# elfi-dev/elfi

Hardware: NVIDIA H100
Metric: accepted particles/sec (higher is better)
Workload: dtype f64

## Files before the change

### elfi_b200/csrc/common.cuh

```cuda
#pragma once

#include <cuda.h>
#include <cuda_runtime.h>

#include <cstdarg>
#include <cstdint>
#include <cstdio>
#include <cstring>

#include "../../include/elfi_b200.h"

namespace elfi {

void set_error(const char* fmt, ...);

#define ELFI_CUDA_OK(expr)                                                              \
    do {                                                                                \
        cudaError_t _e = (expr);                                                        \
        if (_e != cudaSuccess) {                                                        \
            ::elfi::set_error("%s failed: %s (%s:%d)", #expr, cudaGetErrorString(_e),   \
                              __FILE__, __LINE__);                                      \
            cudaGetLastError();       \
            return ELFI_B200_ERR_CUDA;                                                  \
        }                                                                               \
// ... 8 lines not shown
    } while (0)

typedef CUresult (*tensor_map_encode_fn)(CUtensorMap*, CUtensorMapDataType, cuuint32_t, void*,
                                         const cuuint64_t*, const cuuint64_t*,
                                         const cuuint32_t*, const cuuint32_t*,
                                         CUtensorMapInterleave, CUtensorMapSwizzle,
                                         CUtensorMapL2promotion, CUtensorMapFloatOOBfill);

}

struct elfi_b200_ctx {
    int device;
    int sm_count;
    size_t smem_optin;
    elfi::tensor_map_encode_fn encode_tiled;
    void* scratch;
    size_t scratch_bytes;
    void* pinned;
    size_t pinned_bytes;
    void* dev_stage;
    size_t dev_stage_bytes;
    cudaStream_t copy_stream[2];
    cudaEvent_t copy_event[4];
};

namespace elfi {

void* ctx_scratch(elfi_b200_ctx* ctx, size_t bytes);

int make_rowmajor_f64_map(elfi_b200_ctx* ctx, const double* base, int64_t rows, int64_t cols,
                          int64_t ld, int box_rows, CUtensorMap* out);

inline bool tma_compatible(const void* base, int64_t ld) {
    return (reinterpret_cast<uintptr_t>(base) % 16 == 0) && ((ld * 8) % 16 == 0);
}

__device__ __forceinline__ uint32_t smem_u32(const void* p) {
    return static_cast<uint32_t>(__cvta_generic_to_shared(p));
}

__device__ __forceinline__ void mbar_init(uint32_t bar, uint32_t count) {
    asm volatile("mbarrier.init.shared::cta.b64 [%0], %1;" ::"r"(bar), "r"(count) : "memory");
}

__device__ __forceinline__ void mbar_fence_init() {
    asm volatile("fence.mbarrier_init.release.cluster;" ::: "memory");
// ... 25 lines not shown
}

__device__ __forceinline__ void tma_load_2d(uint32_t dst, const CUtensorMap* map, int32_t col0,
                                            int32_t row0, uint32_t bar) {
    asm volatile(
        "cp.async.bulk.tensor.2d.shared::cluster.global.mbarrier::complete_tx::bytes"
        " [%0], [%1, {%2, %3}], [%4];"
        ::"r"(dst), "l"(reinterpret_cast<uint64_t>(map)), "r"(col0), "r"(row0), "r"(bar)
        : "memory");
}

__device__ __forceinline__ void bulk_load_1d(uint32_t dst, const void* src, uint32_t bytes,
                                             uint32_t bar) {
    asm volatile(
        "cp.async.bulk.shared::cluster.global.mbarrier::complete_tx::bytes [%0], [%1], %2, [%3];"
        ::"r"(dst), "l"(src), "r"(bytes), "r"(bar)
        : "memory");
}

__device__ __forceinline__ void tma_prefetch_desc(const CUtensorMap* map) {
    asm volatile("prefetch.tensormap [%0];" ::"l"(reinterpret_cast<uint64_t>(map)) : "memory");
}

}
```

### elfi_b200/csrc/ctx.cu

```cuda
#include "common.cuh"

namespace elfi {

static thread_local char g_error[512] = "";

void set_error(const char* fmt, ...) {
    va_list ap;
    va_start(ap, fmt);
    vsnprintf(g_error, sizeof(g_error), fmt, ap);
    va_end(ap);
}

void* ctx_scratch(elfi_b200_ctx* ctx, size_t bytes) {
    if (bytes <= ctx->scratch_bytes) return ctx->scratch;
    size_t want = bytes + (bytes >> 2) + (1u << 20);
    want = (want + 255) & ~size_t(255);
    if (ctx->scratch) {
        if (cudaDeviceSynchronize() != cudaSuccess || cudaFree(ctx->scratch) != cudaSuccess) {
            set_error("scratch release failed: %s", cudaGetErrorString(cudaGetLastError()));
            ctx->scratch = nullptr;
            ctx->scratch_bytes = 0;
            return nullptr;
        }
        ctx->scratch = nullptr;
// ... 54 lines not shown
        elfi::set_error("ctx_create: device %d is sm_%d%d; this library is built for sm_90a only",
                        device, prop.major, prop.minor);
        return ELFI_B200_ERR_UNSUPPORTED;
    }
    elfi_b200_ctx* ctx = new elfi_b200_ctx();
    memset(ctx, 0, sizeof(*ctx));
    ctx->device = device;
    ctx->sm_count = prop.multiProcessorCount;
    ctx->smem_optin = prop.sharedMemPerBlockOptin;
    void* fn = nullptr;
    cudaDriverEntryPointQueryResult qres;
    cudaError_t e = cudaGetDriverEntryPoint("cuTensorMapEncodeTiled", &fn, cudaEnableDefault, &qres);
    if (e != cudaSuccess || qres != cudaDriverEntryPointSuccess || fn == nullptr) {
        elfi::set_error("ctx_create: cuTensorMapEncodeTiled not available from the driver");
        delete ctx;
        cudaGetLastError();
        return ELFI_B200_ERR_CUDA;
    }
    ctx->encode_tiled = reinterpret_cast<elfi::tensor_map_encode_fn>(fn);
    for (int i = 0; i < 2; ++i)
        ELFI_CUDA_OK(cudaStreamCreateWithFlags(&ctx->copy_stream[i], cudaStreamNonBlocking));
    for (int i = 0; i < 4; ++i)
        ELFI_CUDA_OK(cudaEventCreateWithFlags(&ctx->copy_event[i], cudaEventDisableTiming));
    *out = ctx;
    return ELFI_B200_OK;
}

int elfi_b200_ctx_destroy(elfi_b200_ctx* ctx) {
    if (!ctx) return ELFI_B200_OK;
    cudaSetDevice(ctx->device);
    cudaDeviceSynchronize();
    if (ctx->scratch) cudaFree(ctx->scratch);
    if (ctx->dev_stage) cudaFree(ctx->dev_stage);
    if (ctx->pinned) cudaFreeHost(ctx->pinned);
    for (int i = 0; i < 2; ++i)
        if (ctx->copy_stream[i]) cudaStreamDestroy(ctx->copy_stream[i]);
    for (int i = 0; i < 4; ++i)
        if (ctx->copy_event[i]) cudaEventDestroy(ctx->copy_event[i]);
    delete ctx;
    return ELFI_B200_OK;
}

int elfi_b200_ctx_sm_count(const elfi_b200_ctx* ctx) { return ctx ? ctx->sm_count : 0; }

int elfi_b200_allgather_particles(elfi_b200_ctx* const* ctxs, int64_t n_ctx, const double* const* send,
                                  int64_t rows, int64_t width, double* const* recv,
                                  void* const* streams) {
    ELFI_REQUIRE(ctxs && send && recv && streams && n_ctx >= 1 && n_ctx <= 64,
                 "allgather_particles: bad argument");
    ELFI_REQUIRE(rows >= 0 && width >= 1, "allgather_particles: bad shape");
    for (int64_t g = 0; g < n_ctx; ++g)
        ELFI_REQUIRE(ctxs[g] && (rows == 0 || (send[g] && recv[g])), "allgather_particles: NULL entry %lld",
                     (long long)g);
    if (rows == 0) return ELFI_B200_OK;
    const size_t bytes = size_t(rows) * size_t(width) * 8;
    int caller_device = 0;
    ELFI_CUDA_OK(cudaGetDevice(&caller_device));
// ... 43 lines not shown
```

### elfi_b200/csrc/distance.cu

```cuda
#include <cstdlib>

#include "rowstream.cuh"

extern "C" int elfi_b200_colmoments_f64(elfi_b200_ctx* ctx, const double* S, int64_t ldS, int64_t B,
                                        int64_t D, double* out, void* stream);

namespace elfi {

struct DistParams {
    const double* obs;
    const double* W;
    double* d_out;
    uint32_t* mask;
    int K;
    int has_thr;
    const double* shift_src;
    double* mom_partial;
    const double* thr_dev;
    double thr[ELFI_B200_MAX_NESTED];
    __device__ __forceinline__ double threshold(int k) const {
        return thr_dev ? __ldg(thr_dev + k) : thr[k];
    }
};

// ... 294 lines not shown
                for (int j = 0; j < D; ++j) {
                    const double d = __dsub_rn(__ldg(r + j), __ldg(p.obs + j));
                    acc = __dadd_rn(acc, __dmul_rn(__ldg(w + j), __dmul_rn(d, d)));
                }
            } else {
                for (int j = 0; j < D; ++j) {
                    const double d = __dsub_rn(__ldg(r + j), __ldg(p.obs + j));
                    acc = __dadd_rn(acc, __dmul_rn(d, d));
                }
            }
            const double dist = sqrt(acc);
            p.d_out[row * K + k] = dist;
            if (p.has_thr) ok = ok && (dist <= p.threshold(k));
        }
    }
    if (p.mask != nullptr) {
        const uint32_t bits = __ballot_sync(0xffffffffu, ok && p.has_thr);
        if (lane == 0 && (row - lane) < B) p.mask[row >> 5] = bits;
    }
}

__global__ void __launch_bounds__(1024)
compact_mask_kernel(const uint32_t* __restrict__ mask, int64_t nwords, int64_t B,
                    int32_t* __restrict__ idx, int64_t* __restrict__ n_out) {
    __shared__ int64_t warp_sums[32];
    __shared__ int64_t base_s;
    const int tid = threadIdx.x;
    const int lane = tid & 31;
    const int wid = tid >> 5;
    const int64_t first = int64_t(blockIdx.x) * 1024;

    int64_t before = 0;
    for (int64_t w = tid; w < first; w += 1024) before += __popc(mask[w]);
    for (int o = 16; o > 0; o >>= 1) before += __shfl_xor_sync(0xffffffffu, before, o);
    if (lane == 0) warp_sums[wid] = before;
    __syncthreads();
    if (tid == 0) {
        int64_t t = 0;
        for (int i = 0; i < 32; ++i) t += warp_sums[i];
        base_s = t;
    }
    __syncthreads();
    const int64_t base = base_s;
    __syncthreads();

    const int64_t w = first + tid;
    const uint32_t bits = w < nwords ? mask[w] : 0u;
    const int cnt = __popc(bits);
    int incl = cnt;
    for (int o = 1; o < 32; o <<= 1) {
        const int t = __shfl_up_sync(0xffffffffu, incl, o);
        if (lane >= o) incl += t;
    }
    if (lane == 31) warp_sums[wid] = incl;
    __syncthreads();
    if (wid == 0) {
        int64_t v = warp_sums[lane];
        int64_t inc2 = v;
        for (int o = 1; o < 32; o <<= 1) {
            const int64_t t = __shfl_up_sync(0xffffffffu, inc2, o);
            if (lane >= o) inc2 += t;
        }
        warp_sums[lane] = inc2 - v;
        if (lane == 31 && blockIdx.x == gridDim.x - 1 && n_out != nullptr) *n_out = base + inc2;
    }
    __syncthreads();
    int64_t pos = base + warp_sums[wid] + (incl - cnt);
    if (idx != nullptr) {
        uint32_t b = bits;
        while (b) {
            const int bit = __ffs(b) - 1;
            b &= b - 1;
            idx[pos++] = int32_t(w * 32 + bit);
        }
    }
}

int launch_compact_mask(const uint32_t* mask, int64_t B, int32_t* idx, int64_t* n_out,
                        cudaStream_t stream) {
    const int64_t nwords = (B + 31) / 32;
    if (nwords == 0) {
        if (n_out) ELFI_CUDA_OK(cudaMemsetAsync(n_out, 0, sizeof(int64_t), stream));
        return ELFI_B200_OK;
    }
    const unsigned blocks = unsigned((nwords + 1023) / 1024);
    compact_mask_kernel<<<blocks, 1024, 0, stream>>>(mask, nwords, B, idx, n_out);
    ELFI_CUDA_OK(cudaGetLastError());
    return ELFI_B200_OK;
}

int launch_dist(elfi_b200_ctx* ctx, const double* S, int64_t ldS, int64_t B, int64_t D,
                const double* obs, const double* W, int64_t K, const double* thr_host,
                double* d_out, uint32_t* mask, cudaStream_t stream,
                const double* thr_dev = nullptr) {
    DistParams p;
    memset(&p, 0, sizeof(p));
    p.obs = obs;
    p.W = W;
    p.d_out = d_out;
    p.mask = mask;
    p.K = int(K);
    p.has_thr = thr_host != nullptr || thr_dev != nullptr;
    p.thr_dev = thr_dev;
    if (thr_host)
        for (int k = 0; k < K; ++k) p.thr[k] = thr_host[k];
    if (B == 0) return ELFI_B200_OK;

    const int64_t Dp = ((D + RS_BOX_COLS - 1) / RS_BOX_COLS) * RS_BOX_COLS;
    const bool use_tma = D >= RS_BOX_COLS && tma_compatible(S, ldS);
    if (use_tma) {
// ... 243 lines not shown
    const int64_t Dp = ((D + RS_BOX_COLS - 1) / RS_BOX_COLS) * RS_BOX_COLS;
    const size_t aux = size_t(Dp) * 8 * 2;
    if (D >= RS_BOX_COLS && tma_compatible(S, ldS) && rs_pick_stages(ctx->smem_optin, aux) >= 2)
        return rowstream_launch<SeuclidConsumer>(ctx, S, ldS, B, D, aux, p, stream);
    seuclid_direct_kernel<<<unsigned((B + 255) / 256), 256, 0, stream>>>(S, ldS, B, int(D), p);
    ELFI_CUDA_OK(cudaGetLastError());
    return ELFI_B200_OK;
}

static int check_dist_args(const void* S, int64_t ldS, int64_t B, int64_t D, const void* obs,
                           const void* W, int64_t K, const void* thr, const void* acc_idx) {
    ELFI_REQUIRE(B >= 0 && D >= 1, "dist: bad shape B=%lld D=%lld", (long long)B, (long long)D);
    ELFI_REQUIRE(B == 0 || S != nullptr, "dist: S is NULL");
    ELFI_REQUIRE(obs != nullptr, "dist: obs is NULL");
    ELFI_REQUIRE(ldS >= D, "dist: ldS (%lld) < D (%lld)", (long long)ldS, (long long)D);
    ELFI_REQUIRE(K >= 1 && K <= ELFI_B200_MAX_NESTED, "dist: K=%lld outside [1, %d]",
                 (long long)K, ELFI_B200_MAX_NESTED);
    ELFI_REQUIRE(W != nullptr || K == 1, "dist: K=%lld needs a weight matrix", (long long)K);
    ELFI_REQUIRE(acc_idx == nullptr || thr != nullptr, "dist: acc_idx requires thresholds");
    ELFI_REQUIRE(B < (int64_t(1) << 31), "dist: B must fit int32 row indices");
    return ELFI_B200_OK;
}

}

extern "C" {

int elfi_b200_dist_euclid_thr_f64(elfi_b200_ctx* ctx, const double* S, int64_t ldS, int64_t B,
                                  int64_t D, const double* obs, const double* W, int64_t K,
                                  const double* thr_host, double* d_out, int32_t* acc_idx,
                                  int64_t* n_acc, void* stream_) {
    using namespace elfi;
    ELFI_REQUIRE(ctx != nullptr, "dist: ctx is NULL");
    int rc = check_dist_args(S, ldS, B, D, obs, W, K, thr_host, acc_idx);
    if (rc) return rc;
    ELFI_REQUIRE(B == 0 || d_out != nullptr, "dist: d_out is NULL");
    cudaStream_t stream = static_cast<cudaStream_t>(stream_);
    ELFI_CUDA_OK(cudaSetDevice(ctx->device));
    uint32_t* mask = nullptr;
    if (thr_host != nullptr) {
        const size_t nwords = size_t((B + 31) / 32);
        mask = static_cast<uint32_t*>(ctx_scratch(ctx, nwords * 4 + 256));
        if (!mask) return ELFI_B200_ERR_NOMEM;
    }
    rc = launch_dist(ctx, S, ldS, B, D, obs, W, K, thr_host, d_out, mask, stream);
    if (rc) return rc;
    if (thr_host != nullptr && (acc_idx != nullptr || n_acc != nullptr))
        return launch_compact_mask(mask, B, acc_idx, n_acc, stream);
    return ELFI_B200_OK;
}

int elfi_b200_dist_euclid_thr_dev_f64(elfi_b200_ctx* ctx, const double* S, int64_t ldS, int64_t B,
                                      int64_t D, const double* obs, const double* W, int64_t K,
                                      const double* thr_dev, double* d_out, int32_t* acc_idx,
                                      int64_t* n_acc, void* stream_) {
    using namespace elfi;
    ELFI_REQUIRE(ctx != nullptr && thr_dev != nullptr, "dist: ctx or thr_dev is NULL");
    int rc = check_dist_args(S, ldS, B, D, obs, W, K, thr_dev, acc_idx);
    if (rc) return rc;
    ELFI_REQUIRE(B == 0 || d_out != nullptr, "dist: d_out is NULL");
    cudaStream_t stream = static_cast<cudaStream_t>(stream_);
    ELFI_CUDA_OK(cudaSetDevice(ctx->device));
    const size_t nwords = size_t((B + 31) / 32);
    uint32_t* mask = static_cast<uint32_t*>(ctx_scratch(ctx, nwords * 4 + 256));
    if (!mask) return ELFI_B200_ERR_NOMEM;
    rc = launch_dist(ctx, S, ldS, B, D, obs, W, K, nullptr, d_out, mask, stream, thr_dev);
    if (rc) return rc;
    if (acc_idx != nullptr || n_acc != nullptr)
        return launch_compact_mask(mask, B, acc_idx, n_acc, stream);
    return ELFI_B200_OK;
}

int elfi_b200_dist_euclid_mom_f64(elfi_b200_ctx* ctx, const double* S, int64_t ldS, int64_t B,
                                  int64_t D, const double* obs, const double* W, int64_t K,
                                  const double* thr_host, const double* thr_dev, double* d_out,
                                  int32_t* acc_idx, int64_t* n_acc, double* moments,
                                  void* stream_) {
    using namespace elfi;
    ELFI_REQUIRE(ctx != nullptr && moments != nullptr, "dist_mom: ctx or moments is NULL");
    ELFI_REQUIRE(!(thr_host && thr_dev), "dist_mom: give thresholds on the host OR on the device");
    const void* thr = thr_host ? static_cast<const void*>(thr_host) : thr_dev;
    int rc = check_dist_args(S, ldS, B, D, obs, W, K, thr, acc_idx);
    if (rc) return rc;
    ELFI_REQUIRE(B >= 1 && d_out != nullptr, "dist_mom: needs at least one row and d_out");
    cudaStream_t stream = static_cast<cudaStream_t>(stream_);
    ELFI_CUDA_OK(cudaSetDevice(ctx->device));
    const int64_t Dp = ((D + RS_BOX_COLS - 1) / RS_BOX_COLS) * RS_BOX_COLS;
    const size_t aux = NestedMomentsConsumer<2>::aux_bytes(Dp, K);
    const bool fused = W != nullptr && D >= RS_BOX_COLS && tma_compatible(S, ldS) &&
                       rs_pick_stages(ctx->smem_optin, aux) >= 2;
    const size_t mask_bytes = (size_t((B + 31) / 32) * 4 + 255) & ~size_t(255);
    const size_t part_bytes = fused ? size_t(ctx->sm_count) * 16 * 2 * D * 8 : 0;
    uint8_t* base = static_cast<uint8_t*>(ctx_scratch(ctx, mask_bytes + part_bytes + 256));
// ... 178 lines not shown
```

### elfi_b200/csrc/rowstream.cuh

```cuda
#pragma once

#include <type_traits>

#include "common.cuh"

namespace elfi {

template <class C, class = void> struct rs_has_tile_info : std::false_type {};
template <class C> struct rs_has_tile_info<C, std::void_t<decltype(C::RS_TILE_INFO)>> : std::true_type {};
template <class C, class = void> struct rs_has_finish : std::false_type {};
template <class C> struct rs_has_finish<C, std::void_t<decltype(C::RS_FINISH)>> : std::true_type {};

constexpr int RS_WARPS = 8;
constexpr int RS_BOX_ROWS = 32;
constexpr int RS_BOX_COLS = 16;
constexpr int RS_BOX_BYTES = RS_BOX_ROWS * RS_BOX_COLS * 8;
constexpr int RS_MAX_STAGES = 6;

__host__ __device__ inline size_t rs_box_bytes(int ns, int warps = RS_WARPS) {
    return size_t(warps) * ns * RS_BOX_BYTES;
}
__host__ __device__ inline size_t rs_bar_bytes(int ns, int warps = RS_WARPS) {
    return size_t(warps) * ns * 8;
}
__host__ __device__ inline size_t rs_aux_offset(int ns, int warps = RS_WARPS) {
    return (rs_box_bytes(ns, warps) + rs_bar_bytes(ns, warps) + 15) & ~size_t(15);
}

inline int rs_pick_stages(size_t smem_optin, size_t aux_bytes, int warps = RS_WARPS) {
    for (int ns = RS_MAX_STAGES; ns >= 2; --ns)
        if (rs_aux_offset(ns, warps) + aux_bytes + 1024 <= smem_optin) return ns;
    return 0;
}

template <class Consumer, int WARPS = RS_WARPS>
__global__ void __launch_bounds__(WARPS * 32, 1)
rowstream_kernel(const __grid_constant__ CUtensorMap map, int64_t B, int D, int ns,
                 typename Consumer::Params params) {
    extern __shared__ __align__(1024) uint8_t smem[];
    const int warp = threadIdx.x >> 5;
    const int lane = threadIdx.x & 31;
    uint8_t* aux = smem + rs_aux_offset(ns, WARPS);

    Consumer::setup_shared(aux, params, D);

    const uint32_t box0 = smem_u32(smem) + uint32_t(warp) * ns * RS_BOX_BYTES;
    const uint32_t bar0 = smem_u32(smem + rs_box_bytes(ns, WARPS)) + uint32_t(warp) * ns * 8;
    const uint8_t* box0_generic = smem + size_t(warp) * ns * RS_BOX_BYTES;

    if (lane == 0) {
        if (warp == 0) tma_prefetch_desc(&map);
        for (int s = 0; s < ns; ++s) mbar_init(bar0 + s * 8, 1);
        mbar_fence_init();
    }
    __syncthreads();

    const int Gc = (D + RS_BOX_COLS - 1) / RS_BOX_COLS;
    const int G = Gc * Consumer::PASSES;
    const int64_t ntiles = (B + RS_BOX_ROWS - 1) / RS_BOX_ROWS;
    const int64_t gw = int64_t(blockIdx.x) * WARPS + warp;
    const int64_t GW = int64_t(gridDim.x) * WARPS;
    const int64_t my_tiles = gw < ntiles ? (ntiles - gw + GW - 1) / GW : 0;
    const int64_t nbox = my_tiles * G;

    int64_t p_tile = gw;
    int p_cg = 0;
    int p_col = 0;
    int64_t p_q = 0;
    int p_s = 0;
    auto issue = [&]() {
        mbar_arrive_expect_tx(bar0 + p_s * 8, RS_BOX_BYTES);
        tma_load_2d(box0 + p_s * RS_BOX_BYTES, &map, p_col * RS_BOX_COLS,
                    int32_t(p_tile * RS_BOX_ROWS), bar0 + p_s * 8);
        ++p_q;
        if (++p_s == ns) p_s = 0;
        if (++p_col == Gc) p_col = 0;
        if (++p_cg == G) { p_cg = 0; p_tile += GW; }
// ... 7 lines not shown
    const int sw = lane & 7;
    const uint32_t row_off = uint32_t(lane) * 128;

    int s = 0;
    uint32_t parity = 0;
    int cg = 0;
    int col = 0;
    int pass = 0;
    int64_t tile = gw;
    for (int64_t q = 0; q < nbox; ++q) {
        mbar_wait(bar0 + s * 8, parity);
        if (cg == 0) {
            c.begin_row();
            if constexpr (rs_has_tile_info<Consumer>::value) c.set_tile(tile * RS_BOX_ROWS, B);
        }
        c.consume(pass, col, box0_generic + size_t(s) * RS_BOX_BYTES + row_off, sw);
        __syncwarp();
        if (lane == 0 && p_q < nbox) issue();
        if (cg == G - 1) c.end_row(tile * RS_BOX_ROWS + lane, B, lane);
        if (++col == Gc) { col = 0; ++pass; }
        if (++cg == G) { cg = 0; pass = 0; tile += GW; }
        if (++s == ns) { s = 0; parity ^= 1; }
    }
    if constexpr (rs_has_finish<Consumer>::value) {
        __syncwarp();
        c.finish(gw, lane);
    }
}

template <class Consumer, int WARPS = RS_WARPS>
int rowstream_launch(elfi_b200_ctx* ctx, const double* M, int64_t ld, int64_t B, int64_t D,
                     size_t aux_bytes, const typename Consumer::Params& params,
                     cudaStream_t stream) {
    ELFI_REQUIRE(D <= (int64_t(1) << 30) && B < (int64_t(1) << 31),
                 "matrix too large for int32 TMA coordinates (B=%lld, D=%lld)", (long long)B,
                 (long long)D);
    if (B == 0) return ELFI_B200_OK;
    const int ns = rs_pick_stages(ctx->smem_optin, aux_bytes, WARPS);
    ELFI_REQUIRE(ns >= 2, "row too wide for the shared-memory pipeline (D=%lld)", (long long)D);
    CUtensorMap map;
    int rc = make_rowmajor_f64_map(ctx, M, B, D, ld, RS_BOX_ROWS, &map);
    if (rc) return rc;
    const size_t smem_bytes = rs_aux_offset(ns, WARPS) + aux_bytes;
    auto kern = rowstream_kernel<Consumer, WARPS>;
    ELFI_CUDA_OK(cudaFuncSetAttribute(kern, cudaFuncAttributeMaxDynamicSharedMemorySize,
                                      int(smem_bytes)));
    const int64_t ntiles = (B + RS_BOX_ROWS - 1) / RS_BOX_ROWS;
    int64_t ctas = (ntiles + WARPS - 1) / WARPS;
    if (ctas > ctx->sm_count) ctas = ctx->sm_count;
    kern<<<dim3(unsigned(ctas)), dim3(WARPS * 32), smem_bytes, stream>>>(map, B, int(D), ns, params);
    ELFI_CUDA_OK(cudaGetLastError());
    return ELFI_B200_OK;
}

}
```

### elfi_b200/csrc/select.cu

```cuda
#include <cstdlib>

#include "eqweight.h"
#include "pairwise.cuh"

namespace elfi {

constexpr int SORT_CHUNK = 1024;
constexpr int SORT_WARPS = 8;

__device__ __forceinline__ uint64_t key_to_u64(double d) {
    if (d != d) return ~uint64_t(0);
    uint64_t u = static_cast<uint64_t>(__double_as_longlong(d));
    return (u >> 63) ? ~u : (u | (uint64_t(1) << 63));
}
__device__ __forceinline__ double u64_to_key(uint64_t u) {
    if (u == ~uint64_t(0)) return __longlong_as_double(0x7ff8000000000000LL);
    u = (u >> 63) ? (u & ~(uint64_t(1) << 63)) : ~u;
    return __longlong_as_double(static_cast<long long>(u));
}

__global__ void __launch_bounds__(256)
sort_prepare_kernel(const double* __restrict__ keys, int64_t n, uint64_t* __restrict__ ukeys,
                    int32_t* __restrict__ vals, uint32_t* __restrict__ ghist) {
    __shared__ uint32_t h[8 * 256];
// ... 164 lines not shown
    int cur = 0;
    for (int pass = 0; pass < 8; ++pass) {
        sort_upsweep_kernel<<<wblocks, SORT_WARPS * 32, 0, stream>>>(s.k[cur], n, pass, s.nw, s.ghist, s.whist);
        sort_scan_kernel<<<256, 1024, 0, stream>>>(s.k[cur], n, pass, s.nw, s.ghist, s.whist);
        sort_scatter_kernel<<<wblocks, SORT_WARPS * 32, 0, stream>>>(
            s.k[cur], s.v[cur], n, pass, s.nw, s.ghist, s.whist, s.k[cur ^ 1], s.v[cur ^ 1]);
        cur ^= 1;
    }
    ELFI_CUDA_OK(cudaGetLastError());
    return ELFI_B200_OK;
}

__global__ void __launch_bounds__(256)
gather_rows_kernel(const double* __restrict__ src, int64_t ld_src, const int32_t* __restrict__ idx,
                   int64_t n, int64_t width, double* __restrict__ dst, int64_t ld_dst) {
    const int64_t total = n * width;
    const int64_t stride = int64_t(gridDim.x) * blockDim.x;
    for (int64_t t = int64_t(blockIdx.x) * blockDim.x + threadIdx.x; t < total; t += stride) {
        const int64_t i = t / width, j = t - i * width;
        dst[i * ld_dst + j] = src[int64_t(idx[i]) * ld_src + j];
    }
}

constexpr int APPEND_MAX_SRC = 8;
struct AppendSources {
    const double* ptr[APPEND_MAX_SRC];
    int64_t ld[APPEND_MAX_SRC];
    int32_t width[APPEND_MAX_SRC];
    int32_t col0[APPEND_MAX_SRC];
    int32_t n_src, total_width;
};

__global__ void __launch_bounds__(256)
accept_append_kernel(const int32_t* __restrict__ acc_idx, const int64_t* __restrict__ n_acc,
                     AppendSources src, double* __restrict__ dst, int64_t ld_dst, int64_t capacity,
                     const int64_t* __restrict__ count) {
    const int64_t base = *count;
    int64_t room = capacity - base;
    if (room < 0) room = 0;
    const int64_t rows = *n_acc < room ? *n_acc : room;
    const int64_t total = rows * src.total_width;
    const int64_t stride = int64_t(gridDim.x) * blockDim.x;
    for (int64_t t = int64_t(blockIdx.x) * blockDim.x + threadIdx.x; t < total; t += stride) {
        const int64_t j = t / src.total_width;
        const int c = int(t - j * src.total_width);
        const int64_t row = acc_idx ? int64_t(acc_idx[j]) : j;
        int k = 0;
#pragma unroll
        for (int q = 1; q < APPEND_MAX_SRC; ++q)
            if (q < src.n_src && c >= src.col0[q]) k = q;
        dst[(base + j) * ld_dst + c] = src.ptr[k][row * src.ld[k] + (c - src.col0[k])];
    }
}

__global__ void accept_count_kernel(const int64_t* __restrict__ n_acc, int64_t capacity,
                                    int64_t* __restrict__ count, int64_t* __restrict__ dropped) {
    int64_t room = capacity - *count;
    if (room < 0) room = 0;
    const int64_t rows = *n_acc < room ? *n_acc : room;
    if (dropped) *dropped += *n_acc - rows;
    *count += rows;
}

__global__ void __launch_bounds__(256)
gather2_rows_kernel(const double* __restrict__ A, int64_t ldA, int64_t nA,
                    const double* __restrict__ Bm, int64_t ldB, const int32_t* __restrict__ mapB,
                    const int32_t* __restrict__ perm, int64_t n, int64_t width,
                    double* __restrict__ dst, int64_t ld_dst) {
    const int64_t total = n * width;
    const int64_t stride = int64_t(gridDim.x) * blockDim.x;
    for (int64_t t = int64_t(blockIdx.x) * blockDim.x + threadIdx.x; t < total; t += stride) {
        const int64_t i = t / width, j = t - i * width;
        const int64_t r = perm ? perm[i] : i;
        double v;
        if (r < nA) {
            v = A[r * ldA + j];
        } else {
            const int64_t rb = mapB ? int64_t(mapB[r - nA]) : (r - nA);
            v = Bm[rb * ldB + j];
        }
        dst[i * ld_dst + j] = v;
    }
}

// ... 482 lines not shown
        const int64_t width = width_host[k];
        ELFI_REQUIRE(width >= 1 && dst_host[k] && ld_dst_host[k] >= width &&
                     (nA == 0 || (A_host[k] && ldA_host[k] >= width)) &&
                     (nB == 0 || (B_host[k] && ldB_host[k] >= width)),
                     "topn_merge: bad descriptor of output %lld", (long long)k);
        int64_t gb = (n_keep * width + 255) / 256;
        if (gb > int64_t(ctx->sm_count) * 16) gb = int64_t(ctx->sm_count) * 16;
        gather2_rows_kernel<<<unsigned(gb), 256, 0, stream>>>(A_host[k], ldA_host[k], nA, B_host[k],
                                                              ldB_host[k], mapB, perm, n_keep, width,
                                                              dst_host[k], ld_dst_host[k]);
    }
    ELFI_CUDA_OK(cudaGetLastError());
    return ELFI_B200_OK;
}

int elfi_b200_accept_append_f64(elfi_b200_ctx* ctx, const int32_t* acc_idx, const int64_t* n_acc,
                                int64_t max_rows, int64_t n_src, const double* const* src_host,
                                const int64_t* ld_src_host, const int64_t* width_host, double* dst,
                                int64_t ld_dst, int64_t capacity, int64_t* count, int64_t* dropped,
                                void* stream_) {
    using namespace elfi;
    ELFI_REQUIRE(ctx && n_acc && src_host && ld_src_host && width_host && dst && count,
                 "accept_append: NULL argument");
    ELFI_REQUIRE(n_src >= 1 && n_src <= APPEND_MAX_SRC, "accept_append: 1..%d sources", APPEND_MAX_SRC);
    ELFI_REQUIRE(max_rows >= 0 && capacity >= 0, "accept_append: bad shape");
    AppendSources src;
    memset(&src, 0, sizeof(src));
    src.n_src = int32_t(n_src);
    int64_t col = 0;
    for (int k = 0; k < n_src; ++k) {
        ELFI_REQUIRE(src_host[k] && width_host[k] >= 1 && ld_src_host[k] >= width_host[k],
                     "accept_append: bad source %d", k);
        src.ptr[k] = src_host[k];
        src.ld[k] = ld_src_host[k];
        src.width[k] = int32_t(width_host[k]);
        src.col0[k] = int32_t(col);
        col += width_host[k];
    }
    ELFI_REQUIRE(col <= ld_dst && col < (int64_t(1) << 30), "accept_append: ld_dst < total width");
    src.total_width = int32_t(col);
    if (max_rows == 0) return ELFI_B200_OK;
    cudaStream_t stream = static_cast<cudaStream_t>(stream_);
    ELFI_CUDA_OK(cudaSetDevice(ctx->device));
    int64_t blocks = (max_rows * col + 255) / 256;
    if (blocks > int64_t(ctx->sm_count) * 8) blocks = int64_t(ctx->sm_count) * 8;
    accept_append_kernel<<<unsigned(blocks), 256, 0, stream>>>(acc_idx, n_acc, src, dst, ld_dst,
                                                              capacity, count);
    accept_count_kernel<<<1, 1, 0, stream>>>(n_acc, capacity, count, dropped);
    ELFI_CUDA_OK(cudaGetLastError());
    return ELFI_B200_OK;
}

extern "C" int elfi_b200_dist_euclid_thr_f64(elfi_b200_ctx*, const double*, int64_t, int64_t, int64_t,
                                             const double*, const double*, int64_t, const double*,
                                             double*, int32_t*, int64_t*, void*);
extern "C" int elfi_b200_dist_euclid_thr_dev_f64(elfi_b200_ctx*, const double*, int64_t, int64_t,
                                                 int64_t, const double*, const double*, int64_t,
                                                 const double*, double*, int32_t*, int64_t*, void*);

int elfi_b200_rejection_batch_f64(elfi_b200_ctx* ctx, const double* S, int64_t ldS, int64_t B,
                                  int64_t D, const double* obs, const double* W, int64_t K,
                                  const double* thr_host, const double* thr_dev, double* d_out,
                                  int32_t* acc_idx, int64_t* n_acc, int64_t n_extra,
                                  const double* const* extra_host, const int64_t* ld_extra_host,
                                  const int64_t* width_extra_host, double* dst, int64_t ld_dst,
                                  int64_t capacity, int64_t* count, int64_t* dropped,
                                  void* stream_) {
    using namespace elfi;
    ELFI_REQUIRE(ctx && acc_idx && n_acc && d_out, "rejection_batch: NULL argument");
    ELFI_REQUIRE((thr_host != nullptr) != (thr_dev != nullptr),
                 "rejection_batch: thresholds on the host OR on the device");
    ELFI_REQUIRE(n_extra >= 0 && n_extra < APPEND_MAX_SRC, "rejection_batch: 0..%d extra sources",
                 APPEND_MAX_SRC - 1);
    int rc = thr_host
        ? elfi_b200_dist_euclid_thr_f64(ctx, S, ldS, B, D, obs, W, K, thr_host, d_out, acc_idx, n_acc,
                                        stream_)
        : elfi_b200_dist_euclid_thr_dev_f64(ctx, S, ldS, B, D, obs, W, K, thr_dev, d_out, acc_idx,
                                            n_acc, stream_);
    if (rc) return rc;
    const double* src[APPEND_MAX_SRC];
    int64_t ld[APPEND_MAX_SRC], width[APPEND_MAX_SRC];
    src[0] = d_out; ld[0] = K; width[0] = K;
    for (int64_t k = 0; k < n_extra; ++k) {
        src[k + 1] = extra_host[k];
        ld[k + 1] = ld_extra_host[k];
        width[k + 1] = width_extra_host[k];
    }
    return elfi_b200_accept_append_f64(ctx, acc_idx, n_acc, B, n_extra + 1, src, ld, width, dst,
                                       ld_dst, capacity, count, dropped, stream_);
}

int elfi_b200_wquantile_f64(elfi_b200_ctx* ctx, const double* x, const double* w, int64_t n,
                            double alpha, double* out, void* stream_) {
    using namespace elfi;
    ELFI_REQUIRE(ctx != nullptr && x != nullptr && out != nullptr, "wquantile: NULL argument");
    ELFI_REQUIRE(n >= 1 && n < (int64_t(1) << 31), "wquantile: n=%lld out of range", (long long)n);
    ELFI_REQUIRE(alpha >= 0.0 && alpha <= 1.0, "wquantile: alpha=%g outside [0, 1]", alpha);
    cudaStream_t stream = static_cast<cudaStream_t>(stream_);
    ELFI_CUDA_OK(cudaSetDevice(ctx->device));
    const size_t sort_bytes = sort_scratch_bytes(n);
    const size_t extra = align256(size_t(n + 2) * 8) + 256;
    uint8_t* base = static_cast<uint8_t*>(ctx_scratch(ctx, sort_bytes + extra));
    if (!base) return ELFI_B200_ERR_NOMEM;
    SortScratch s = carve_sort(base, n);
    double* ws = reinterpret_cast<double*>(base + sort_bytes);
    double* total = reinterpret_cast<double*>(base + sort_bytes + align256(size_t(n) * 8));
    int rc = sort_pairs_device(x, n, s, ctx->sm_count, stream);
    if (rc) return rc;
    if (w == nullptr && alpha > 0.0) {
        wq_pick_kernel<<<1, 1, 0, stream>>>(s.k[0], equal_weight_cum_index(n, alpha) - 1, out);
        ELFI_CUDA_OK(cudaGetLastError());
        return ELFI_B200_OK;
// ... 62 lines not shown
```

Baseline: 26.29 million.

## Fuse accept-append into compaction kernel and chain launches with PDL

The rejection batch path now does the append of accepted rows inside the mask-compaction kernel. Each CTA copies its own span of accepted rows, and the last CTA, found with a global ticket counter, commits the count. This removes the separate append and count kernels. The distance and compaction kernels are launched with programmatic dependent launch so their prologues can overlap the previous kernel. The standalone append also merges its count kernel into a last-CTA commit. The cost is a ticket atomic, a cross-CTA read of n_out through a volatile load, and append work placed on the compaction CTAs. That last part could add imbalance or small-grid underutilisation.

```diff
diff --git a/elfi_b200/csrc/append.cuh b/elfi_b200/csrc/append.cuh
--- /dev/null
+++ b/elfi_b200/csrc/append.cuh
@@ -0,0 +1,93 @@
+#pragma once
+
+#include "common.cuh"
+
+namespace elfi {
+
+constexpr int APPEND_MAX_SRC = 8;
+struct AppendSources {
+    const double* ptr[APPEND_MAX_SRC];
+    int64_t ld[APPEND_MAX_SRC];
+    int32_t width[APPEND_MAX_SRC];
+    int32_t col0[APPEND_MAX_SRC];
+    int32_t n_src, total_width;
+};
+
+struct AppendJob {
+    AppendSources src;
+    double* dst;
+    int64_t ld_dst;
+    int64_t capacity;
+    int64_t* count;
+    int64_t* dropped;
+};
+
+inline int append_sources(int64_t n_src, const double* const* src_host, const int64_t* ld_host,
+                          const int64_t* width_host, int64_t ld_dst, AppendSources* out) {
+    ELFI_REQUIRE(n_src >= 1 && n_src <= APPEND_MAX_SRC, "accept_append: 1..%d sources", APPEND_MAX_SRC);
+    memset(out, 0, sizeof(*out));
+    out->n_src = int32_t(n_src);
+    int64_t col = 0;
+    for (int k = 0; k < n_src; ++k) {
+        ELFI_REQUIRE(src_host[k] && width_host[k] >= 1 && ld_host[k] >= width_host[k],
+                     "accept_append: bad source %d", k);
+        out->ptr[k] = src_host[k];
+        out->ld[k] = ld_host[k];
+        out->width[k] = int32_t(width_host[k]);
+        out->col0[k] = int32_t(col);
+        col += width_host[k];
+    }
+    ELFI_REQUIRE(col <= ld_dst && col < (int64_t(1) << 30), "accept_append: ld_dst < total width");
+    out->total_width = int32_t(col);
+    return ELFI_B200_OK;
+}
+
+__device__ __forceinline__ int64_t append_rows(const AppendJob& a, int64_t base, int64_t n) {
+    int64_t room = a.capacity - base;
+    if (room < 0) room = 0;
+    return n < room ? n : room;
+}
+
+__device__ __forceinline__ void append_element(const AppendJob& a, int64_t base, int64_t j,
+                                               int64_t row, int c) {
+    int k = 0;
+#pragma unroll
+    for (int q = 1; q < APPEND_MAX_SRC; ++q)
+        if (q < a.src.n_src && c >= a.src.col0[q]) k = q;
+    a.dst[(base + j) * a.ld_dst + c] = a.src.ptr[k][row * a.src.ld[k] + (c - a.src.col0[k])];
+}
+
+__device__ __forceinline__ void append_span(const AppendJob& a, int64_t base,
+                                            const int32_t* acc_idx, int64_t j0, int64_t n,
+                                            int64_t t0, int64_t stride) {
+    const int w = a.src.total_width;
+    const int64_t total = append_rows(a, base + j0, n) * w;
+    for (int64_t t = t0; t < total; t += stride) {
+        const int64_t j = j0 + t / w;
+        append_element(a, base, j, acc_idx ? int64_t(acc_idx[j]) : j, int(t % w));
+    }
+}
+
+__device__ __forceinline__ bool append_last_cta(unsigned int* ticket) {
+    __shared__ bool last_s;
+    __syncthreads();
+    if (threadIdx.x == 0) {
+        __threadfence();
+        const unsigned int t = atomicAdd(ticket, 1u);
+        last_s = t == gridDim.x - 1;
+        if (last_s) {
+            __threadfence();
+            *ticket = 0u;
+        }
+    }
+    __syncthreads();
+    return last_s;
+}
+
+__device__ __forceinline__ void append_commit(const AppendJob& a, int64_t base, int64_t n) {
+    const int64_t rows = append_rows(a, base, n);
+    if (a.dropped) *a.dropped += n - rows;
+    *a.count = base + rows;
+}
+
+}
diff --git a/elfi_b200/csrc/common.cuh b/elfi_b200/csrc/common.cuh
--- a/elfi_b200/csrc/common.cuh
+++ b/elfi_b200/csrc/common.cuh
@@ -54,6 +54,7 @@
     size_t dev_stage_bytes;
     cudaStream_t copy_stream[2];
     cudaEvent_t copy_event[4];
+    unsigned int* ticket;
 };
 
 namespace elfi {
@@ -125,4 +126,27 @@
     asm volatile("prefetch.tensormap [%0];" ::"l"(reinterpret_cast<uint64_t>(map)) : "memory");
 }
 
+__device__ __forceinline__ void grid_dep_wait() {
+    asm volatile("griddepcontrol.wait;" ::: "memory");
 }
+__device__ __forceinline__ void grid_dep_launch_dependents() {
+    asm volatile("griddepcontrol.launch_dependents;" ::: "memory");
+}
+
+template <typename... KernelArgs, typename... Args>
+cudaError_t launch_pdl(void (*kernel)(KernelArgs...), dim3 grid, dim3 block, size_t smem,
+                       cudaStream_t stream, Args&&... args) {
+    cudaLaunchAttribute attr[1];
+    attr[0].id = cudaLaunchAttributeProgrammaticStreamSerialization;
+    attr[0].val.programmaticStreamSerializationAllowed = 1;
+    cudaLaunchConfig_t cfg = {};
+    cfg.gridDim = grid;
+    cfg.blockDim = block;
+    cfg.dynamicSmemBytes = smem;
+    cfg.stream = stream;
+    cfg.attrs = attr;
+    cfg.numAttrs = 1;
+    return cudaLaunchKernelEx(&cfg, kernel, static_cast<Args&&>(args)...);
+}
+
+}
diff --git a/elfi_b200/csrc/ctx.cu b/elfi_b200/csrc/ctx.cu
--- a/elfi_b200/csrc/ctx.cu
+++ b/elfi_b200/csrc/ctx.cu
@@ -100,6 +100,8 @@
         ELFI_CUDA_OK(cudaStreamCreateWithFlags(&ctx->copy_stream[i], cudaStreamNonBlocking));
     for (int i = 0; i < 4; ++i)
         ELFI_CUDA_OK(cudaEventCreateWithFlags(&ctx->copy_event[i], cudaEventDisableTiming));
+    ELFI_CUDA_OK(cudaMalloc(&ctx->ticket, 256));
+    ELFI_CUDA_OK(cudaMemset(ctx->ticket, 0, 256));
     *out = ctx;
     return ELFI_B200_OK;
 }
@@ -111,6 +113,7 @@
     if (ctx->scratch) cudaFree(ctx->scratch);
     if (ctx->dev_stage) cudaFree(ctx->dev_stage);
     if (ctx->pinned) cudaFreeHost(ctx->pinned);
+    if (ctx->ticket) cudaFree(ctx->ticket);
     for (int i = 0; i < 2; ++i)
         if (ctx->copy_stream[i]) cudaStreamDestroy(ctx->copy_stream[i]);
     for (int i = 0; i < 4; ++i)
diff --git a/elfi_b200/csrc/distance.cu b/elfi_b200/csrc/distance.cu
--- a/elfi_b200/csrc/distance.cu
+++ b/elfi_b200/csrc/distance.cu
@@ -1,5 +1,6 @@
 #include <cstdlib>
 
+#include "append.cuh"
 #include "rowstream.cuh"
 
 extern "C" int elfi_b200_colmoments_f64(elfi_b200_ctx* ctx, const double* S, int64_t ldS, int64_t B,
@@ -340,13 +341,18 @@
 
 __global__ void __launch_bounds__(1024)
 compact_mask_kernel(const uint32_t* __restrict__ mask, int64_t nwords, int64_t B,
-                    int32_t* __restrict__ idx, int64_t* __restrict__ n_out) {
+                    int32_t* __restrict__ idx, int64_t* __restrict__ n_out, AppendJob app,
+                    unsigned int* __restrict__ ticket) {
     __shared__ int64_t warp_sums[32];
-    __shared__ int64_t base_s;
+    __shared__ int64_t base_s, cta_count_s;
     const int tid = threadIdx.x;
     const int lane = tid & 31;
     const int wid = tid >> 5;
     const int64_t first = int64_t(blockIdx.x) * 1024;
+
+    grid_dep_wait();
+    grid_dep_launch_dependents();
+    const int64_t fill = app.dst != nullptr ? *app.count : 0;
 
     int64_t before = 0;
     for (int64_t w = tid; w < first; w += 1024) before += __popc(mask[w]);
@@ -380,7 +386,13 @@
             if (lane >= o) inc2 += t;
         }
         warp_sums[lane] = inc2 - v;
-        if (lane == 31 && blockIdx.x == gridDim.x - 1 && n_out != nullptr) *n_out = base + inc2;
+        if (lane == 31) {
+            cta_count_s = inc2;
+            if (blockIdx.x == gridDim.x - 1 && n_out != nullptr) {
+                *n_out = base + inc2;
+                __threadfence();
+            }
+        }
     }
     __syncthreads();
     int64_t pos = base + warp_sums[wid] + (incl - cnt);
@@ -392,18 +404,28 @@
             idx[pos++] = int32_t(w * 32 + bit);
         }
     }
+    if (app.dst != nullptr) {
+        __syncthreads();
+        append_span(app, fill, idx, base, cta_count_s, tid, blockDim.x);
+        if (append_last_cta(ticket) && tid == 0)
+            append_commit(app, fill, *reinterpret_cast<volatile int64_t*>(n_out));
+    }
 }
 
 int launch_compact_mask(const uint32_t* mask, int64_t B, int32_t* idx, int64_t* n_out,
-                        cudaStream_t stream) {
+                        cudaStream_t stream, const AppendJob* app = nullptr,
+                        unsigned int* ticket = nullptr) {
     const int64_t nwords = (B + 31) / 32;
     if (nwords == 0) {
         if (n_out) ELFI_CUDA_OK(cudaMemsetAsync(n_out, 0, sizeof(int64_t), stream));
         return ELFI_B200_OK;
     }
+    AppendJob job;
+    memset(&job, 0, sizeof(job));
+    if (app != nullptr) job = *app;
     const unsigned blocks = unsigned((nwords + 1023) / 1024);
-    compact_mask_kernel<<<blocks, 1024, 0, stream>>>(mask, nwords, B, idx, n_out);
-    ELFI_CUDA_OK(cudaGetLastError());
+    ELFI_CUDA_OK(launch_pdl(compact_mask_kernel, dim3(blocks), dim3(1024), 0, stream, mask, nwords,
+                            B, idx, n_out, job, ticket));
     return ELFI_B200_OK;
 }
 
@@ -693,6 +715,29 @@
     return ELFI_B200_OK;
 }
 
+static int dist_thr(elfi_b200_ctx* ctx, const double* S, int64_t ldS, int64_t B, int64_t D,
+                    const double* obs, const double* W, int64_t K, const double* thr_host,
+                    const double* thr_dev, double* d_out, int32_t* acc_idx, int64_t* n_acc,
+                    const AppendJob* app, cudaStream_t stream) {
+    const void* thr_any = thr_host ? static_cast<const void*>(thr_host) : thr_dev;
+    const bool thr = thr_any != nullptr;
+    int rc = check_dist_args(S, ldS, B, D, obs, W, K, thr_any, acc_idx);
+    if (rc) return rc;
+    ELFI_REQUIRE(B == 0 || d_out != nullptr, "dist: d_out is NULL");
+    ELFI_CUDA_OK(cudaSetDevice(ctx->device));
+    uint32_t* mask = nullptr;
+    if (thr) {
+        const size_t nwords = size_t((B + 31) / 32);
+        mask = static_cast<uint32_t*>(ctx_scratch(ctx, nwords * 4 + 256));
+        if (!mask) return ELFI_B200_ERR_NOMEM;
+    }
+    rc = launch_dist(ctx, S, ldS, B, D, obs, W, K, thr_host, d_out, mask, stream, thr_dev);
+    if (rc) return rc;
+    if (thr && (acc_idx != nullptr || n_acc != nullptr || app != nullptr))
+        return launch_compact_mask(mask, B, acc_idx, n_acc, stream, app, ctx->ticket);
+    return ELFI_B200_OK;
+}
+
 }
 
 extern "C" {
@@ -703,22 +748,8 @@
                                   int64_t* n_acc, void* stream_) {
     using namespace elfi;
     ELFI_REQUIRE(ctx != nullptr, "dist: ctx is NULL");
-    int rc = check_dist_args(S, ldS, B, D, obs, W, K, thr_host, acc_idx);
-    if (rc) return rc;
-    ELFI_REQUIRE(B == 0 || d_out != nullptr, "dist: d_out is NULL");
-    cudaStream_t stream = static_cast<cudaStream_t>(stream_);
-    ELFI_CUDA_OK(cudaSetDevice(ctx->device));
-    uint32_t* mask = nullptr;
-    if (thr_host != nullptr) {
-        const size_t nwords = size_t((B + 31) / 32);
-        mask = static_cast<uint32_t*>(ctx_scratch(ctx, nwords * 4 + 256));
-        if (!mask) return ELFI_B200_ERR_NOMEM;
-    }
-    rc = launch_dist(ctx, S, ldS, B, D, obs, W, K, thr_host, d_out, mask, stream);
-    if (rc) return rc;
-    if (thr_host != nullptr && (acc_idx != nullptr || n_acc != nullptr))
-        return launch_compact_mask(mask, B, acc_idx, n_acc, stream);
-    return ELFI_B200_OK;
+    return dist_thr(ctx, S, ldS, B, D, obs, W, K, thr_host, nullptr, d_out, acc_idx, n_acc, nullptr,
+                    static_cast<cudaStream_t>(stream_));
 }
 
 int elfi_b200_dist_euclid_thr_dev_f64(elfi_b200_ctx* ctx, const double* S, int64_t ldS, int64_t B,
@@ -727,19 +758,45 @@
                                       int64_t* n_acc, void* stream_) {
     using namespace elfi;
     ELFI_REQUIRE(ctx != nullptr && thr_dev != nullptr, "dist: ctx or thr_dev is NULL");
-    int rc = check_dist_args(S, ldS, B, D, obs, W, K, thr_dev, acc_idx);
-    if (rc) return rc;
-    ELFI_REQUIRE(B == 0 || d_out != nullptr, "dist: d_out is NULL");
-    cudaStream_t stream = static_cast<cudaStream_t>(stream_);
-    ELFI_CUDA_OK(cudaSetDevice(ctx->device));
-    const size_t nwords = size_t((B + 31) / 32);
-    uint32_t* mask = static_cast<uint32_t*>(ctx_scratch(ctx, nwords * 4 + 256));
-    if (!mask) return ELFI_B200_ERR_NOMEM;
-    rc = launch_dist(ctx, S, ldS, B, D, obs, W, K, nullptr, d_out, mask, stream, thr_dev);
-    if (rc) return rc;
-    if (acc_idx != nullptr || n_acc != nullptr)
-        return launch_compact_mask(mask, B, acc_idx, n_acc, stream);
-    return ELFI_B200_OK;
+    return dist_thr(ctx, S, ldS, B, D, obs, W, K, nullptr, thr_dev, d_out, acc_idx, n_acc, nullptr,
+                    static_cast<cudaStream_t>(stream_));
+}
+
+int elfi_b200_rejection_batch_f64(elfi_b200_ctx* ctx, const double* S, int64_t ldS, int64_t B,
+                                  int64_t D, const double* obs, const double* W, int64_t K,
+                                  const double* thr_host, const double* thr_dev, double* d_out,
+                                  int32_t* acc_idx, int64_t* n_acc, int64_t n_extra,
+                                  const double* const* extra_host, const int64_t* ld_extra_host,
+                                  const int64_t* width_extra_host, double* dst, int64_t ld_dst,
+                                  int64_t capacity, int64_t* count, int64_t* dropped,
+                                  void* stream_) {
+    using namespace elfi;
+    ELFI_REQUIRE(ctx && acc_idx && n_acc && d_out, "rejection_batch: NULL argument");
+    ELFI_REQUIRE((thr_host != nullptr) != (thr_dev != nullptr),
+                 "rejection_batch: thresholds on the host OR on the device");
+    ELFI_REQUIRE(n_extra >= 0 && n_extra < APPEND_MAX_SRC, "rejection_batch: 0..%d extra sources",
+                 APPEND_MAX_SRC - 1);
+    ELFI_REQUIRE(dst && count && (n_extra == 0 || (extra_host && ld_extra_host && width_extra_host)),
+                 "accept_append: NULL argument");
+    ELFI_REQUIRE(capacity >= 0, "accept_append: bad shape");
+    const double* src[APPEND_MAX_SRC];
+    int64_t ld[APPEND_MAX_SRC], width[APPEND_MAX_SRC];
+    src[0] = d_out; ld[0] = K; width[0] = K;
+    for (int64_t k = 0; k < n_extra; ++k) {
+        src[k + 1] = extra_host[k];
+        ld[k + 1] = ld_extra_host[k];
+        width[k + 1] = width_extra_host[k];
+    }
+    AppendJob app;
+    int rc = append_sources(n_extra + 1, src, ld, width, ld_dst, &app.src);
+    if (rc) return rc;
+    app.dst = dst;
+    app.ld_dst = ld_dst;
+    app.capacity = capacity;
+    app.count = count;
+    app.dropped = dropped;
+    return dist_thr(ctx, S, ldS, B, D, obs, W, K, thr_host, thr_dev, d_out, acc_idx, n_acc, &app,
+                    static_cast<cudaStream_t>(stream_));
 }
 
 int elfi_b200_dist_euclid_mom_f64(elfi_b200_ctx* ctx, const double* S, int64_t ldS, int64_t B,
diff --git a/elfi_b200/csrc/rowstream.cuh b/elfi_b200/csrc/rowstream.cuh
--- a/elfi_b200/csrc/rowstream.cuh
+++ b/elfi_b200/csrc/rowstream.cuh
@@ -42,8 +42,6 @@
     const int lane = threadIdx.x & 31;
     uint8_t* aux = smem + rs_aux_offset(ns, WARPS);
 
-    Consumer::setup_shared(aux, params, D);
-
     const uint32_t box0 = smem_u32(smem) + uint32_t(warp) * ns * RS_BOX_BYTES;
     const uint32_t bar0 = smem_u32(smem + rs_box_bytes(ns, WARPS)) + uint32_t(warp) * ns * 8;
     const uint8_t* box0_generic = smem + size_t(warp) * ns * RS_BOX_BYTES;
@@ -53,6 +51,9 @@
         for (int s = 0; s < ns; ++s) mbar_init(bar0 + s * 8, 1);
         mbar_fence_init();
     }
+    grid_dep_wait();
+
+    Consumer::setup_shared(aux, params, D);
     __syncthreads();
 
     const int Gc = (D + RS_BOX_COLS - 1) / RS_BOX_COLS;
@@ -106,6 +107,7 @@
         if (++cg == G) { cg = 0; pass = 0; tile += GW; }
         if (++s == ns) { s = 0; parity ^= 1; }
     }
+    grid_dep_launch_dependents();
     if constexpr (rs_has_finish<Consumer>::value) {
         __syncwarp();
         c.finish(gw, lane);
@@ -132,8 +134,8 @@
     const int64_t ntiles = (B + RS_BOX_ROWS - 1) / RS_BOX_ROWS;
     int64_t ctas = (ntiles + WARPS - 1) / WARPS;
     if (ctas > ctx->sm_count) ctas = ctx->sm_count;
-    kern<<<dim3(unsigned(ctas)), dim3(WARPS * 32), smem_bytes, stream>>>(map, B, int(D), ns, params);
-    ELFI_CUDA_OK(cudaGetLastError());
+    ELFI_CUDA_OK(launch_pdl(kern, dim3(unsigned(ctas)), dim3(WARPS * 32), smem_bytes, stream, map, B,
+                            int(D), ns, params));
     return ELFI_B200_OK;
 }
 
diff --git a/elfi_b200/csrc/select.cu b/elfi_b200/csrc/select.cu
--- a/elfi_b200/csrc/select.cu
+++ b/elfi_b200/csrc/select.cu
@@ -1,5 +1,6 @@
 #include <cstdlib>
 
+#include "append.cuh"
 #include "eqweight.h"
 #include "pairwise.cuh"
 
@@ -210,44 +211,14 @@
     }
 }
 
-constexpr int APPEND_MAX_SRC = 8;
-struct AppendSources {
-    const double* ptr[APPEND_MAX_SRC];
-    int64_t ld[APPEND_MAX_SRC];
-    int32_t width[APPEND_MAX_SRC];
-    int32_t col0[APPEND_MAX_SRC];
-    int32_t n_src, total_width;
-};
-
 __global__ void __launch_bounds__(256)
 accept_append_kernel(const int32_t* __restrict__ acc_idx, const int64_t* __restrict__ n_acc,
-                     AppendSources src, double* __restrict__ dst, int64_t ld_dst, int64_t capacity,
-                     const int64_t* __restrict__ count) {
-    const int64_t base = *count;
-    int64_t room = capacity - base;
-    if (room < 0) room = 0;
-    const int64_t rows = *n_acc < room ? *n_acc : room;
-    const int64_t total = rows * src.total_width;
-    const int64_t stride = int64_t(gridDim.x) * blockDim.x;
-    for (int64_t t = int64_t(blockIdx.x) * blockDim.x + threadIdx.x; t < total; t += stride) {
-        const int64_t j = t / src.total_width;
-        const int c = int(t - j * src.total_width);
-        const int64_t row = acc_idx ? int64_t(acc_idx[j]) : j;
-        int k = 0;
-#pragma unroll
-        for (int q = 1; q < APPEND_MAX_SRC; ++q)
-            if (q < src.n_src && c >= src.col0[q]) k = q;
-        dst[(base + j) * ld_dst + c] = src.ptr[k][row * src.ld[k] + (c - src.col0[k])];
-    }
-}
-
-__global__ void accept_count_kernel(const int64_t* __restrict__ n_acc, int64_t capacity,
-                                    int64_t* __restrict__ count, int64_t* __restrict__ dropped) {
-    int64_t room = capacity - *count;
-    if (room < 0) room = 0;
-    const int64_t rows = *n_acc < room ? *n_acc : room;
-    if (dropped) *dropped += *n_acc - rows;
-    *count += rows;
+                     AppendJob app, unsigned int* __restrict__ ticket) {
+    const int64_t base = *app.count;
+    const int64_t n = *n_acc;
+    append_span(app, base, acc_idx, 0, n, int64_t(blockIdx.x) * blockDim.x + threadIdx.x,
+                int64_t(gridDim.x) * blockDim.x);
+    if (append_last_cta(ticket) && threadIdx.x == 0) append_commit(app, base, n);
 }
 
 __global__ void __launch_bounds__(256)
@@ -776,72 +747,25 @@
     using namespace elfi;
     ELFI_REQUIRE(ctx && n_acc && src_host && ld_src_host && width_host && dst && count,
                  "accept_append: NULL argument");
-    ELFI_REQUIRE(n_src >= 1 && n_src <= APPEND_MAX_SRC, "accept_append: 1..%d sources", APPEND_MAX_SRC);
     ELFI_REQUIRE(max_rows >= 0 && capacity >= 0, "accept_append: bad shape");
-    AppendSources src;
-    memset(&src, 0, sizeof(src));
-    src.n_src = int32_t(n_src);
-    int64_t col = 0;
-    for (int k = 0; k < n_src; ++k) {
-        ELFI_REQUIRE(src_host[k] && width_host[k] >= 1 && ld_src_host[k] >= width_host[k],
-                     "accept_append: bad source %d", k);
-        src.ptr[k] = src_host[k];
-        src.ld[k] = ld_src_host[k];
-        src.width[k] = int32_t(width_host[k]);
-        src.col0[k] = int32_t(col);
-        col += width_host[k];
-    }
-    ELFI_REQUIRE(col <= ld_dst && col < (int64_t(1) << 30), "accept_append: ld_dst < total width");
-    src.total_width = int32_t(col);
+    AppendJob app;
+    int rc = append_sources(n_src, src_host, ld_src_host, width_host, ld_dst, &app.src);
+    if (rc) return rc;
+    app.dst = dst;
+    app.ld_dst = ld_dst;
+    app.capacity = capacity;
+    app.count = count;
+    app.dropped = dropped;
     if (max_rows == 0) return ELFI_B200_OK;
     cudaStream_t stream = static_cast<cudaStream_t>(stream_);
     ELFI_CUDA_OK(cudaSetDevice(ctx->device));
-    int64_t blocks = (max_rows * col + 255) / 256;
+    const int64_t bound = max_rows < capacity ? max_rows : capacity;
+    int64_t blocks = (bound * app.src.total_width + 255) / 256;
     if (blocks > int64_t(ctx->sm_count) * 8) blocks = int64_t(ctx->sm_count) * 8;
-    accept_append_kernel<<<unsigned(blocks), 256, 0, stream>>>(acc_idx, n_acc, src, dst, ld_dst,
-                                                              capacity, count);
-    accept_count_kernel<<<1, 1, 0, stream>>>(n_acc, capacity, count, dropped);
+    if (blocks < 1) blocks = 1;
+    accept_append_kernel<<<unsigned(blocks), 256, 0, stream>>>(acc_idx, n_acc, app, ctx->ticket);
     ELFI_CUDA_OK(cudaGetLastError());
     return ELFI_B200_OK;
-}
-
-extern "C" int elfi_b200_dist_euclid_thr_f64(elfi_b200_ctx*, const double*, int64_t, int64_t, int64_t,
-                                             const double*, const double*, int64_t, const double*,
-                                             double*, int32_t*, int64_t*, void*);
-extern "C" int elfi_b200_dist_euclid_thr_dev_f64(elfi_b200_ctx*, const double*, int64_t, int64_t,
-                                                 int64_t, const double*, const double*, int64_t,
-                                                 const double*, double*, int32_t*, int64_t*, void*);
-
-int elfi_b200_rejection_batch_f64(elfi_b200_ctx* ctx, const double* S, int64_t ldS, int64_t B,
-                                  int64_t D, const double* obs, const double* W, int64_t K,
-                                  const double* thr_host, const double* thr_dev, double* d_out,
-                                  int32_t* acc_idx, int64_t* n_acc, int64_t n_extra,
-                                  const double* const* extra_host, const int64_t* ld_extra_host,
-                                  const int64_t* width_extra_host, double* dst, int64_t ld_dst,
-                                  int64_t capacity, int64_t* count, int64_t* dropped,
-                                  void* stream_) {
-    using namespace elfi;
-    ELFI_REQUIRE(ctx && acc_idx && n_acc && d_out, "rejection_batch: NULL argument");
-    ELFI_REQUIRE((thr_host != nullptr) != (thr_dev != nullptr),
-                 "rejection_batch: thresholds on the host OR on the device");
-    ELFI_REQUIRE(n_extra >= 0 && n_extra < APPEND_MAX_SRC, "rejection_batch: 0..%d extra sources",
-                 APPEND_MAX_SRC - 1);
-    int rc = thr_host
-        ? elfi_b200_dist_euclid_thr_f64(ctx, S, ldS, B, D, obs, W, K, thr_host, d_out, acc_idx, n_acc,
-                                        stream_)
-        : elfi_b200_dist_euclid_thr_dev_f64(ctx, S, ldS, B, D, obs, W, K, thr_dev, d_out, acc_idx,
-                                            n_acc, stream_);
-    if (rc) return rc;
-    const double* src[APPEND_MAX_SRC];
-    int64_t ld[APPEND_MAX_SRC], width[APPEND_MAX_SRC];
-    src[0] = d_out; ld[0] = K; width[0] = K;
-    for (int64_t k = 0; k < n_extra; ++k) {
-        src[k + 1] = extra_host[k];
-        ld[k + 1] = ld_extra_host[k];
-        width[k + 1] = width_extra_host[k];
-    }
-    return elfi_b200_accept_append_f64(ctx, acc_idx, n_acc, B, n_extra + 1, src, ld, width, dst,
-                                       ld_dst, capacity, count, dropped, stream_);
 }
 
 int elfi_b200_wquantile_f64(elfi_b200_ctx* ctx, const double* x, const double* w, int64_t n,
```

Result: no change. 26.60 million (median of 6 runs) (+1.2%).
